# AIRI-Institute/nablaDFT

Measured on AMD Instinct MI355X. Metric: conformer-steps/sec (fwd+bwd) + MAE(E,F) vs CPU reference, higher is better.
Workload: dtype f32 (dense products >= 192 tiles: f32 values split exactly into 3 bf16 pieces, 6 MFMA piece products, f32 accumulate; non-finite operands give NaN where plain f32 gives inf); 1 GPU; PaiNN-OC (nablaDFT/painn_pyg, config/model/painn-oc.yaml: F=128 L=6 R=100 rc=5A K=100) energy+forces train step incl. neighbour list, L1+L2 loss, grad all-reduce, clip 5.0, AdamW lr 5e-4; synthetic ~42-atom drug-like conformers, 2048 conformers/GPU/step; conformers_per_gpu=2048, edges_last_step=1737976, parallelism=dp1

## Files before the change

include/nablaq.h:

```cpp
#ifndef NABLAQ_H
#define NABLAQ_H
#include <stddef.h>
#include <stdint.h>

#ifdef __cplusplus
extern "C" {
#endif

#define NQ_OK 0
#define NQ_ERR_HIP 1
#define NQ_ERR_ARG 2
#define NQ_ERR_MOL_TOO_LARGE 3
#define NQ_ERR_WORKSPACE 4
#define NQ_ERR_NO_EDGES 5

#define NQ_ABI_VERSION 17

typedef struct nq_painn_cfg {
  int32_t hidden_channels;
  int32_t num_layers;
  int32_t num_rbf;
  int32_t num_elements;
  int32_t max_neighbors;
  int32_t envelope_exponent;
// ... 295 lines not shown
void nq_profile_enable(int32_t on);
int nq_profile_read(char* names_host, int32_t name_stride, double* total_ms_host, int64_t* counts_host, int32_t cap);
int nq_profile_read2(char* names_host, int32_t name_stride, double* total_ms_host, int64_t* counts_host, double* flops_host, int32_t cap);

void nq_set_gemm_variant(int32_t variant);
void nq_gemm_splitk_release(void);
int nq_gemm_splitk_state(void* stream, uint64_t* ptr, uint64_t* floats, int32_t* captured, int32_t* retired);

int nq_linear_forward(const float* A, const float* W, const float* bias, float* C, float* C_silu, int32_t M, int32_t N, int32_t K,
                      void* stream);
int nq_linear_forward_act(const float* A, const float* W, float* C, float* C_act, const float* resid, float alpha, float beta, int32_t M, int32_t N,
                          int32_t K, void* stream);
int nq_linear_forward_res(const float* A, const float* W, const float* aux, float alpha, float* C, int32_t M, int32_t N, int32_t K, void* stream);
int nq_bf16_pack(const float* W, int32_t N, int32_t K, void* Wb, void* WbT, void* stream);
int nq_linear_forward_bf16(const float* A, const void* Wb, float* C, float* C_act, const float* resid, float alpha, float beta, int32_t M, int32_t N,
                           int32_t K, void* stream);
int nq_linear_input_grad_bf16(const float* G, const void* WbT, float* C, int32_t M, int32_t N, int32_t K, int32_t accumulate, void* stream);
size_t nq_weight_grad_bf16_scratch_bytes(int64_t rows, int32_t N, int32_t K);
int nq_linear_weight_grad_bf16(const float* G, const float* X, float* gW, int64_t rows, int32_t N, int32_t K, void* scratch, void* stream);
int nq_linear_forward_bf16_out(const void* A, int32_t a_bf16, const void* Wb, void* pre_bf16, void* act, int32_t act_bf16, const float* resid, float alpha,
                               float beta, int32_t M, int32_t N, int32_t K, void* stream);
int nq_linear_weight_grad_bf16_x(const float* G, const void* X_bf16, float* gW, int64_t rows, int32_t N, int32_t K, void* scratch, void* stream);
int nq_gn_ssilu_backward_bf16(const void* z_bf16, const float* g, float scale, int64_t n, float* out, void* stream);
int nq_linear_input_grad(const float* G, const float* W, float* C, int32_t M, int32_t N, int32_t K, int32_t accumulate, void* stream);
int nq_linear_input_grad_epi(const float* G, const float* W, float* C, int32_t M, int32_t N, int32_t K, const float* aux, float alpha, float beta, int32_t mode,
                             void* stream);
int nq_linear_input_grad_bf16_epi(const float* G, const void* WbT, float* C, int32_t M, int32_t N, int32_t K, const float* aux, float alpha, float beta,
                                  int32_t mode, void* stream);
size_t nq_column_sum_scratch_floats(int64_t rows, int32_t cols);
int nq_column_sum(const float* A, int64_t rows, int32_t cols, int64_t lda, float* out, float* scratch, void* stream);
size_t nq_weight_grad_scratch_floats(int64_t rows, int32_t N, int32_t K);
int nq_linear_weight_grad(const float* G, const float* X, float* gW, int64_t rows, int32_t N, int32_t K, float* scratch, void* stream);
int nq_linear_weight_grad_bias(const float* G, const float* X, float* gW, float* gb, int64_t rows, int32_t N, int32_t K, float* scratch, void* stream);

int nq_rccl_available(void);
int nq_rccl_unique_id(void* id128);
int nq_rccl_comm_create(const void* id128, int32_t world, int32_t rank, void** comm);
int nq_rccl_comm_destroy(void* comm);
int nq_rccl_comm_count(void* comm, int32_t* count);
int nq_allreduce(float* buf, size_t n, void* comm, void* stream);
int nq_allreduce_mean(float* buf, size_t n, void* comm, void* stream);
int nq_rccl_broadcast(float* buf, size_t n, int32_t root, void* comm, void* stream);

size_t nq_lbfgs_state_bytes(int32_t N, int32_t B, int32_t memory);
int nq_lbfgs_state_layout(int32_t N, int32_t B, int32_t memory, size_t* offsets_host);
int nq_lbfgs_init(void* state, size_t state_bytes, const int32_t* mol_ptr_host, int32_t N, int32_t B, int32_t memory, const void* pos, int32_t pos_f64,
                  float* pos32, int32_t* n_small_host, void* stream);
int nq_lbfgs_step(void* state, int32_t N, int32_t B, int32_t memory, int32_t n_small, const void* forces, int32_t forces_f64, const uint8_t* fixed_mask,
                  float* pos32, double fmax, double maxstep, double damping, double alpha, int32_t evaluate_only, void* stream);

int nq_md_constants(double* kappa_kb_host);
size_t nq_md_state_bytes(int32_t N, int32_t B, int32_t log_cap, int32_t frame_cap, int32_t flags);
int nq_md_state_layout(int32_t N, int32_t B, int32_t log_cap, int32_t frame_cap, int32_t flags, size_t* offsets_host);
int nq_md_init(void* state, size_t state_bytes, const int32_t* mol_ptr_host, const int64_t* mol_key_host, const double* masses_host, const uint8_t* fixed_host,
               int32_t N, int32_t B, int32_t log_cap, int32_t frame_cap, int32_t flags, const void* pos, int32_t pos_f64, const double* vel, float* pos32,
               int32_t* n_small_host, void* stream);
int nq_md_init_velocities(void* state, int32_t N, int32_t B, int32_t n_small, int32_t log_cap, int32_t frame_cap, int32_t flags, double T_init, int64_t seed,
                          int32_t remove_translation, int32_t remove_rotation, void* stream);
int nq_md_step(void* state, int32_t N, int32_t B, int32_t n_small, int32_t log_cap, int32_t frame_cap, int32_t flags, const void* forces, int32_t forces_f64,
               const void* energies, int32_t energies_f64, float* pos32, int32_t mode, double dt, double kT, double fr, int32_t interval, int64_t seed,
               const double* xi, const double* eta, int32_t finish_only, void* stream);
int nq_md_normals(int64_t seed, int32_t step, int32_t draw, const int32_t* mol_ptr, const int64_t* mol_key, int32_t N, int32_t B, double* out, void* stream);

size_t nq_vib_state_bytes(int32_t N, int32_t B, int32_t D, int64_t P);
int nq_vib_state_layout(int32_t N, int32_t B, int32_t D, int64_t P, size_t* offsets_host);
int nq_vib_init(void* state, size_t state_bytes, const int32_t* mol_ptr_host, const double* masses_host, const uint8_t* fixed_host, int32_t N, int32_t B,
// ... 83 lines not shown
```

nabladft_amd/_lib.py:

```python
import ctypes as C
import os

import torch

_HERE = os.path.dirname(os.path.abspath(__file__))
LIB_PATH = os.environ.get("NABLAQ_LIB") or os.path.join(_HERE, "libnablaq.so")
ABI_VERSION = 17

NQ_OK, NQ_ERR_HIP, NQ_ERR_ARG, NQ_ERR_MOL_TOO_LARGE, NQ_ERR_WORKSPACE, NQ_ERR_NO_EDGES = range(6)


class NablaqError(RuntimeError):
    def __init__(self, code, msg):
        super().__init__(f"libnablaq error {code}: {msg}")
        self.code = code


class PainnCfg(C.Structure):
    _fields_ = [("hidden_channels", C.c_int32), ("num_layers", C.c_int32), ("num_rbf", C.c_int32),
                ("num_elements", C.c_int32), ("max_neighbors", C.c_int32), ("envelope_exponent", C.c_int32),
                ("cutoff", C.c_double), ("rbf_coeff", C.c_float), ("filter_mode", C.c_int32), ("rbf_type", C.c_int32), ("reserved", C.c_int32)]


class SchnetCfg(C.Structure):
# ... 139 lines not shown
    "nq_rowop_blocks": (C.c_int, [_P, _I64, _P, _I64, _P, _I32, _I32, _P, _P, _I64, _I32, _I32, _I32, _I32, _I32, _P]),
    "nq_s2_activation_blocks": (C.c_int, [_P, _P, _I32, _I32, _I32, _I64, _I32, _P, _P, _P, _P, _I32, _P]),
    "nq_column_sum_scratch_floats": (_SZ, [_I64, _I32]),
    "nq_column_sum": (C.c_int, [_P, _I64, _I32, _I64, _P, _P, _P]),
    "nq_es_rotate": (C.c_int, [_P, _I64, _P, _I64, _P, _I32, _P, _P, _I32, _I32, _I64, _P, _I32, _I32, _I32, _P]),
    "nq_es_rotate_back": (C.c_int, [_P, _I64, _I32, _P, _P, _I32, _I32, _P, _P, _P, _P, _I64, _P, _I32, _I32, _I32, _P]),
    "nq_eq_layernorm_forward": (C.c_int, [_P, _I64, _P, _P, _I64, _I32, _F, _P, _I64, _P, _P]),
    "nq_eq_layernorm_scratch_floats": (_SZ, [_I64, _I32]),
    "nq_eq_layernorm_backward": (C.c_int, [_P, _I64, _P, _P, _I64, _P, _I64, _I32, _P, _I64, _P, _P, _P, _P]),
    "nq_eq_norm_sh_forward": (C.c_int, [_P, _P, _P, _P, _P, _I64, _I32, _I32, _F, _P, _P, _P]),
    "nq_eq_norm_sh_scratch_floats": (_SZ, [_I64, _I32, _I32]),
    "nq_eq_norm_sh_backward": (C.c_int, [_P, _P, _P, _P, _P, _P, _I64, _I32, _I32, _P, _P, _P, _P, _P, _P]),
    "nq_eq_logits_forward": (C.c_int, [_P, _P, _I64, _I32, _I32, _P, _P]),
    "nq_eq_logits_scratch_floats": (_SZ, [_I64, _I32, _I32]),
    "nq_eq_logits_backward": (C.c_int, [_P, _P, _P, _I64, _I32, _I32, _P, _P, _P, _P]),
    "nq_eq_softmax_forward": (C.c_int, [_P, _P, _I64, _I32, _P, _P]),
    "nq_eq_softmax_backward": (C.c_int, [_P, _P, _P, _I64, _I32, _P, _P]),
    "nq_eq_head_scale": (C.c_int, [_I32, _P, _P, _P, _P, _I64, _I32, _I32, _P, _P, _P]),
    "nq_eq_scale": (C.c_int, [_P, _P, _P, _P, _I64, _I32, _I32, _P, _P]),
    "nq_loss_l1_l2": (C.c_int, [_P, _P, _I32, _P, _P, _I32, _F, _F, _P, _P, _P, _P]),
    "nq_loss_mse": (C.c_int, [_P, _P, _I32, _P, _P, _I32, _F, _F, _P, _P, _P, _P]),
    "nq_adamw_step": (C.c_int, [_P, _P, _P, _P, _SZ, _F, _F, _F, _F, _F, _F, _I32, _P, _P]),
    "nq_profile_enable": (None, [_I32]),
    "nq_profile_read": (C.c_int, [C.c_char_p, _I32, C.POINTER(C.c_double), C.POINTER(C.c_int64), _I32]),
    "nq_profile_read2": (C.c_int, [C.c_char_p, _I32, C.POINTER(C.c_double), C.POINTER(C.c_int64), C.POINTER(C.c_double), _I32]),
    "nq_set_gemm_variant": (None, [_I32]),
    "nq_gemm_splitk_release": (None, []),
    "nq_gemm_splitk_state": (C.c_int, [_P, C.POINTER(C.c_uint64), C.POINTER(C.c_uint64), C.POINTER(C.c_int32), C.POINTER(C.c_int32)]),
    "nq_linear_forward": (C.c_int, [_P, _P, _P, _P, _P, _I32, _I32, _I32, _P]),
    "nq_linear_input_grad": (C.c_int, [_P, _P, _P, _I32, _I32, _I32, _I32, _P]),
    "nq_weight_grad_scratch_floats": (_SZ, [_I64, _I32, _I32]),
    "nq_linear_weight_grad": (C.c_int, [_P, _P, _P, _I64, _I32, _I32, _P, _P]),
    "nq_linear_weight_grad_bias": (C.c_int, [_P, _P, _P, _P, _I64, _I32, _I32, _P, _P]),
    "nq_rccl_available": (C.c_int, []),
    "nq_rccl_unique_id": (C.c_int, [_P]),
    "nq_rccl_comm_create": (C.c_int, [_P, _I32, _I32, C.POINTER(C.c_void_p)]),
    "nq_rccl_comm_destroy": (C.c_int, [_P]),
    "nq_rccl_comm_count": (C.c_int, [_P, C.POINTER(C.c_int32)]),
    "nq_allreduce": (C.c_int, [_P, _SZ, _P, _P]),
    "nq_allreduce_mean": (C.c_int, [_P, _SZ, _P, _P]),
    "nq_rccl_broadcast": (C.c_int, [_P, _SZ, _I32, _P, _P]),
    "nq_lbfgs_state_bytes": (_SZ, [_I32, _I32, _I32]),
    "nq_lbfgs_state_layout": (C.c_int, [_I32, _I32, _I32, C.POINTER(_SZ)]),
    "nq_lbfgs_init": (C.c_int, [_P, _SZ, _P, _I32, _I32, _I32, _P, _I32, _P, C.POINTER(C.c_int32), _P]),
    "nq_lbfgs_step": (C.c_int, [_P, _I32, _I32, _I32, _I32, _P, _I32, _P, _P, _D, _D, _D, _D, _I32, _P]),
    "nq_md_constants": (C.c_int, [C.POINTER(C.c_double)]),
    "nq_md_state_bytes": (_SZ, [_I32, _I32, _I32, _I32, _I32]),
    "nq_md_state_layout": (C.c_int, [_I32, _I32, _I32, _I32, _I32, C.POINTER(_SZ)]),
    "nq_md_init": (C.c_int, [_P, _SZ, _P, _P, _P, _P, _I32, _I32, _I32, _I32, _I32, _P, _I32, _P, _P, C.POINTER(C.c_int32), _P]),
    "nq_md_init_velocities": (C.c_int, [_P, _I32, _I32, _I32, _I32, _I32, _I32, _D, _I64, _I32, _I32, _P]),
    "nq_md_step": (C.c_int, [_P, _I32, _I32, _I32, _I32, _I32, _I32, _P, _I32, _P, _I32, _P, _I32, _D, _D, _D, _I32, _I64, _P, _P, _I32, _P]),
    "nq_md_normals": (C.c_int, [_I64, _I32, _I32, _P, _P, _I32, _I32, _P, _P]),
    "nq_vib_state_bytes": (_SZ, [_I32, _I32, _I32, _I64]),
    "nq_vib_state_layout": (C.c_int, [_I32, _I32, _I32, _I64, C.POINTER(_SZ)]),
    "nq_vib_init": (C.c_int, [_P, _SZ, _P, _P, _P, _I32, _I32, _I32, _I64, _P, _I32, C.POINTER(C.c_int32), _P]),
    "nq_vib_displace": (C.c_int, [_P, _I32, _I32, _I32, _I64, _I32, _I32, _D, _P, _I64, _P]),
    "nq_vib_accumulate": (C.c_int, [_P, _I32, _I32, _I32, _I64, _I32, _I32, _P, _I32, _I64, _P]),
    "nq_vib_finish": (C.c_int, [_P, _I32, _I32, _I32, _I64, _P]),
    "nq_vib_eigh": (C.c_int, [_P, _I32, _I32, _I32, _I64, _I32, _I32, _I32, _I32, _P]),
    "nq_g3d_max_mol_atoms": (C.c_int32, []),
    "nq_g3d_pair_forward": (C.c_int, [_P] * 9 + [_I32, _I32, _I32, _P, _P, _P, _P, _P]),
    "nq_g3d_pair_scratch_floats": (_SZ, [_I32, _I64, _I32]),
    "nq_g3d_pair_backward": (C.c_int, [_P] * 12 + [_I32, _I64, _I32] + [_P] * 8),
    "nq_g3d_bias_to_heads": (C.c_int, [_P, _P, _P, _P, _I32, _I32, _P, _P]),
    "nq_g3d_bias_from_heads": (C.c_int, [_P, _P, _P, _P, _I32, _I32, _P, _P]),
    "nq_g3d_attention_forward": (C.c_int, [_P, _P, _P, _F, _P, _P, _I32, _I32, _I32, _I32, _I32, _F, _P, _P, _P]),
# ... 106 lines not shown
```

nabladft_amd/build.py:

```python
import os
import subprocess
import sys

HERE = os.path.dirname(os.path.abspath(__file__))
CSRC = os.path.join(HERE, "csrc")
OBJ = os.path.join(HERE, "csrc", "_obj")
LIB = os.path.join(HERE, "libnablaq.so")
SOURCES = ["graph.hip", "gemm.hip", "gemm_bf16.hip", "edge.hip", "molpair.hip", "updfuse.hip", "node.hip", "schnet.hip", "hblock.hip", "so3.hip", "qhnet.hip", "qhgen.hip", "gemnet_graph.hip", "gemnet.hip", "escn.hip", "equiformer.hip", "geobasis.hip", "graphormer.hip", "dimenet.hip", "lbfgs.hip", "md.hip", "vib.hip", "rccl.hip", "engine.hip"]
EXTRA = {"molpair.hip": ["-fno-slp-vectorize"], "md.hip": ["-ffp-contract=off"], "vib.hip": ["-ffp-contract=off"]}
FLAGS = ["--offload-arch=gfx950", "-O3", "-std=c++17", "-fPIC", "-fno-fast-math", "-ffp-contract=on", "-Wall", "-Wno-unused-function"]


def _newer(target, deps):
    if not os.path.exists(target):
        return True
    t = os.path.getmtime(target)
    return any(os.path.getmtime(d) > t for d in deps)


def build(force=False, verbose=True):
    hipcc = os.environ.get("HIPCC", "/opt/rocm/bin/hipcc")
    os.makedirs(OBJ, exist_ok=True)
    headers = [os.path.join(CSRC, "common.h"), os.path.join(CSRC, "lanes.h"), os.path.join(CSRC, "gemm_tile.h"), os.path.join(CSRC, "gemm_split.h"), os.path.join(CSRC, "cg_l4.inc"), os.path.join(os.path.dirname(HERE), "include", "nablaq.h")]
    objs, procs = [], []
    for s in SOURCES:
        src, obj = os.path.join(CSRC, s), os.path.join(OBJ, s.replace(".hip", ".o"))
        objs.append(obj)
        if force or _newer(obj, [src] + headers):
            cmd = [hipcc] + FLAGS + EXTRA.get(s, []) + ["-c", src, "-o", obj]
            if verbose:
                print(" ".join(cmd), flush=True)
            procs.append((s, subprocess.Popen(cmd, stdout=subprocess.PIPE, stderr=subprocess.STDOUT, text=True)))
    failed = False
    for s, p in procs:
        out, _ = p.communicate()
        if out.strip() and verbose:
            print(out)
        if p.returncode != 0:
            print(f"hipcc failed on {s}:\n{out}", file=sys.stderr)
            failed = True
    if failed:
        raise RuntimeError("hipcc compilation failed")
    if force or procs or _newer(LIB, objs):
        cmd = [hipcc, "--offload-arch=gfx950", "-shared", "-fPIC", "-o", LIB] + objs
        if verbose:
            print(" ".join(cmd), flush=True)
        subprocess.check_call(cmd)
    return LIB


if __name__ == "__main__":
    build(force="--force" in sys.argv)
    print("built", LIB)
```

nabladft_amd/csrc/engine.hip:

```cpp
#include <stdarg.h>
#include <stdlib.h>
#include <string.h>

#include "../../include/nablaq.h"
#include "common.h"

thread_local char nq_err_buf[512] = "";
int nq_fail(int code, const char* fmt, ...) {
  va_list ap;
  va_start(ap, fmt);
  vsnprintf(nq_err_buf, sizeof(nq_err_buf), fmt, ap);
  va_end(ap);
  return code;
}

#include <map>
#include <mutex>
#include <utility>
static std::mutex g_lds_mu;
static std::map<std::pair<int, const void*>, size_t> g_lds_granted;
int nq_dyn_lds(const void* kernel, size_t bytes) {
  int dev = 0;
  NQ_HIP(hipGetDevice(&dev));
  std::lock_guard<std::mutex> lock(g_lds_mu);
// ... 93 lines not shown
    y.Z1 = take(2 * N * F); y.Hh = take(2 * N * F); y.XH = take(2 * N * 3 * F);
    y.PHI = take(EP * 3 * F); y.PSI = take(EP * 3 * F); y.WRT = take(R * 3 * F);
    y.XM = take(2 * N * F); y.VM = take(2 * N * 3 * F); y.UU = take(2 * N * 6 * F);
    y.S = take(2 * N * F); y.CAT = take(2 * N * 2 * F); y.ZQ = take(2 * N * F); y.Q = take(2 * N * F); y.Y = take(2 * N * 3 * F);
    y.UFRAG = take(nq_updfuse_frag_floats((int)F));
    const size_t st_ = W->fused ? 1 : 0;
    y.LGY = take(st_ * 2 * N * 3 * F); y.LGCAT = take(st_ * 2 * N * 2 * F); y.LGU = take(st_ * 2 * N * 6 * F); y.LGXH = take(st_ * 2 * N * 3 * F);
    y.LGXA = take(st_ * N * F); y.LGXB = take(st_ * N * F); y.LGVA = take(st_ * N * 3 * F); y.LGVB = take(st_ * N * 3 * F);
    y.LGQ = take(st_ * 2 * N * F); y.LGH = take(st_ * 2 * N * F); y.LGQP = take(st_ * N * F); y.LGHP = take(st_ * N * F);
  }
  W->RHO2 = take(2 * EP * R);
  W->ORDER = take(W->fused ? E : 0);
  W->RW = take(W->fused ? E * 32 : 0);
  W->ZO = take(2 * N * H); W->e_atom = take(N); W->te_atom = take(N);
  W->TD = take(E); W->TR = take(3 * E); W->pos_dot = take(3 * N); W->ge = take(N); W->gte = take(N);
  W->GX = take(2 * N * F); W->GVa = take(2 * N * 3 * F); W->GVb = take(2 * N * 3 * F);
  W->GY = take(2 * N * 3 * F); W->GQ = take(2 * N * F); W->GCAT = take(2 * N * 2 * F); W->GU = take(2 * N * 6 * F);
  W->GXH = take(2 * N * 3 * F); W->GH = take(2 * N * F);
  W->GBR = take(N * 3 * F);
  W->GPHI2 = take(2 * E * 3 * F);
  W->GEDGE = take((F / 64) * E * 4);
  W->GZO = take(2 * N * H); W->TMPW = take(N * H);
  W->GRHO = take(c->rbf_type ? 2 * E * R : 0); W->BCON = take(c->rbf_type ? E * R : 0);
  W->ROWCTR = take(5 * L * NQ_ROWCTR_INTS);
  W->SCHED = take(W->fused ? nq_molgw_sched_ints((int)E, (int)B) : 0);
  W->GWREC = take(W->fused ? nq_molgw_rec_floats((int)E, (int)B) : 0);
  W->GWPART = take(W->fused ? nq_molgw_part_floats((int)F, (int)B) : 0);
  size_t s = 0;
  auto mx = [&](size_t v) { if (v > s) s = v; };
  mx(nq_gemm_tn_scratch_floats(2 * N, 3 * F, F)); mx(nq_gemm_tn_scratch_floats(2 * N, F, 2 * F)); mx(nq_gemm_tn_scratch_floats(6 * N, 2 * F, F));
  mx(W->fused ? nq_gwr_scratch_floats((int)E, (int)F, (int)R) : nq_gemm_tn_scratch_floats(2 * E, 3 * F, R));
  if (W->fused) mx(nq_k0_sort_scratch_ints((int)E, (int)R));
  mx(nq_gemm_tn_scratch_floats(2 * N, F, F)); mx(nq_gemm_tn_scratch_floats(2 * N, H, F));
  mx(nq_colsum_scratch_floats(N > E ? N : E, 3 * F));
  if (c->rbf_type) { mx(nq_colsum_scratch_floats(E, R)); mx(nq_colsum_scratch_floats(E * R, 1)); }
  mx(nq_embed_grad_scratch_floats((int)N, (int)F, (int)T));
  W->scratch_floats = s;
  W->scratch = take(s);
  W->total_floats = o;
  (void)B;
}

enum { GW_PAIR_ROWS = 0, GW_MOLECULE = 1, GW_MIXED = 2 };
struct StepPlan {
  bool fused;
  int gw_mode, gw_cap;
  bool lite;
  bool fused_update;
  bool layer0;
  bool top_layer;
  bool side_fwd, side_geom, side_reduce;
  bool geom_rev_serial;
};
static StepPlan plan_step(const nq_painn_cfg* c, const nq_graph* g, bool want_forces) {
  auto env_on = [](const char* name) { const char* v = getenv(name); return v && v[0] == '1'; };
  StepPlan p{};
  p.fused = c->rbf_type == 0 && nq_filter_fits_lds(c->hidden_channels, c->num_rbf) && !env_on("NQ_NO_FUSED_FILTER");
  const char* cap = getenv("NQ_MOLGW_CAP");
  const int hw = nq_molgw_max_atoms();
  p.gw_cap = cap && atoi(cap) > 0 && atoi(cap) < hw ? atoi(cap) : hw;
  p.gw_mode = GW_PAIR_ROWS;
  if (p.fused && !env_on("NQ_NO_MOLGW") && nq_molgw_config_ok(c->hidden_channels, c->num_rbf) && g->max_mol_atoms > 0 && (env_on("NQ_MOLGW") || g->N >= 4096))
    p.gw_mode = g->max_mol_atoms <= p.gw_cap ? GW_MOLECULE : GW_MIXED;
  p.lite = p.fused && want_forces && !env_on("NQ_NO_LITE");
  p.fused_update = nq_updfuse_frag_floats(c->hidden_channels) > 0 && !env_on("NQ_NO_FUSED_UPDATE") && !nq_gemm_exact_f32_requested();
  p.layer0 = !env_on("NQ_NO_LAYER0");
// ... 520 lines not shown
  NQ_TRY(nq_gemm_nn(st, ws + W.GZO, params + P.O1, ws + W.GX, lite ? N : 2 * N, H, F, H, F, F, 0, "O1"));
  float* gv_cur = ws + W.GVa; float* gv_oth = ws + W.GVb;
  const bool top_layer = plan.top_layer && !seeded;
  if (!top_layer) NQ_HIP(hipMemsetAsync(gv_cur, 0, (lite ? 3 : 6) * NF * sizeof(float), st));
  if (seeded) {
    if (seed_x) NQ_TRY(nq_axpy(st, seed_x, ws + W.GX, (long)NF));
    if (seed_vec) NQ_HIP(hipMemcpyAsync(gv_cur, seed_vec, 3 * NF * sizeof(float), hipMemcpyDeviceToDevice, st));
  }
  float* gphi = ws + W.GPHI2; float* gpsi = gphi + (size_t)E * 3 * F;
  const int* const n_big_pairs = sched + nq_molgw_sched_ints(E, g.B) - 1;
  if (molgw && !geom_aside) NQ_TRY(nq_molgw_geometry(st, g, ws + W.RW, ws + W.TD, ws + W.TR, sched, ws + W.GWREC));
  if (geom_aside) ss.main_waits(geom_ready);
  if (mixed) NQ_HIP(hipMemsetAsync(ws + W.GBR, 0, 3 * NF * sizeof(float), st));
  for (int l = L - 1; l >= 0; --l) {
    const WsLayer& y = W.lay[l]; const MsgP& mp = P.msg[l]; const UpdP& up = P.upd[l];
    const bool top = top_layer && l == L - 1;
    const bool l0 = plan.layer0 && l == 0;
    float* const GYs = lite ? ws + y.LGY : ws + W.GY;
    float* const GCATs = lite ? ws + y.LGCAT : ws + W.GCAT;
    float* const GUs = lite ? ws + y.LGU : ws + W.GU;
    float* const GXHs = lite ? ws + y.LGXH : ws + W.GXH;
    float* const GQs = lite ? ws + y.LGQ : ws + W.GQ;
    float* const GHs = lite ? ws + y.LGH : ws + W.GH;
    UpdRevArgs u{};
    u.N = N; u.F = F; u.U = ws + y.UU; u.Y = ws + y.Y; u.S = ws + y.S; u.CAT = ws + y.CAT;
    u.TU = ws + y.UU + 6 * NF; u.TY = ws + y.Y + 3 * NF; u.TS = ws + y.S + NF; u.TCAT = ws + y.CAT + 2 * NF;
    u.GX = ws + W.GX; u.GTX = lite ? ws + y.LGXA : ws + W.GX + NF; u.GV = gv_cur; u.GTV = lite ? ws + y.LGVA : gv_cur + 3 * NF;
    u.GY = GYs; u.GTY = GYs + 3 * NF; u.GCAT = GCATs; u.GTCAT = GCATs + 2 * NF;
    u.GU = GUs; u.GTU = GUs + 6 * NF;
    u.lite = lite ? 1 : 0;
    ss.before_main_writes(SB_GY);
    NQ_TRY(nq_upd_rev(st, u, 1, true, top));
    sd = ss.fork();
    NQ_TRY(nq_gemm_tn(sd, GYs, ws + y.Q, gp + up.V2, 2L * N, 3 * F, F, 3 * F, F, scr, "V2", gp + up.c2, N));
    ss.read_by_side(SB_GY);
    ss.before_main_writes(SB_GQ);
    NQ_TRY(nq_gemm_nn(st, GYs, params + up.V2, GQs, lite ? N : 2 * N, top ? 2 * F : 3 * F, F, 3 * F, F, F, 0, "V2"));
    NQ_TRY(nq_silu_rev(st, ws + y.ZQ, ws + y.ZQ + NF, GQs, lite ? ws + y.LGQP : GQs + NF, (long)NF, true, lite));
    sd = ss.fork();
    NQ_TRY(nq_gemm_tn(sd, GQs, ws + y.CAT, gp + up.V1, 2L * N, F, 2 * F, F, 2 * F, scr, "V1", gp + up.c1, N));
    ss.read_by_side(SB_GQ);
    NQ_TRY(nq_gemm_nn(st, GQs, params + up.V1, GCATs, lite ? N : 2 * N, F, 2 * F, F, 2 * F, 2 * F, 0, "V1"));
    ss.before_main_writes(SB_GU);
    NQ_TRY(nq_upd_rev(st, u, 2, true, top));
    sd = ss.fork();
    NQ_TRY(nq_gemm_tn(sd, GUs, ws + y.VM, gp + up.U, 6L * N, 2 * F, F, 2 * F, F, scr, "U"));
    ss.read_by_side(SB_GU);
    NQ_TRY(nq_gemm_nn(st, GUs, params + up.U, gv_cur, lite ? 3 * N : 6 * N, 2 * F, F, 2 * F, F, F, top ? 0 : 1, "U"));
    MsgRevArgs m{};
    m.g = g; m.F = F; m.V = ws + W.V[l]; m.XH = ws + y.XH; m.PHI = ws + y.PHI; m.PSI = ws + y.PSI;
    m.TV = ws + W.V[l] + 3 * NF; m.TXH = ws + y.XH + 3 * NF; m.TD = ws + W.TD; m.TR = ws + W.TR;
    m.GX = ws + W.GX; m.GV = gv_cur; m.GTX = lite ? ws + y.LGXB : ws + W.GX + NF; m.GTV = lite ? ws + y.LGVB : gv_cur + 3 * NF;
    m.GXH = GXHs; m.GTXH = GXHs + 3 * NF; m.GV_out = gv_oth; m.GTV_out = gv_oth + 3 * NF;
    m.lite = lite ? 1 : 0;
    m.GPHI = gphi; m.GPSI = gpsi; m.GBR = ws + W.GBR;
    ss.before_main_writes(SB_GXH); ss.before_main_writes(SB_GPHI); ss.before_main_writes(SB_GBR);
    if (W.fused) {
      FilterArgs fa;
      nq_make_filter_args(&fa, ws + y.WRT, params + mp.br, rbf_offsets, ws + W.RW, R, cfg->cutoff, cfg->envelope_exponent, cfg->rbf_coeff, cfg->filter_mode);
      fa.row_ctr = row_ctr(3, l);
      m.mol_cap = plan.gw_cap;
      m.row_filter = mixed ? 1 : 0;
      NQ_TRY(nq_msgf_rev(st, m, fa, true, !molgw, l0));
      if (mixed) {
        m.row_filter = 2;
        fa.row_ctr = row_ctr(4, l);
        NQ_TRY(nq_msgf_rev(st, m, fa, true, true));
// ... 94 lines not shown
```

nabladft_amd/csrc/gemm.hip:

```cpp
#include <algorithm>
#include <map>
#include <mutex>
#include <vector>
#include "gemm_tile.h"
#include "gemm_split.h"

#define BM 128
#define BN 128

__device__ __forceinline__ long rm_row(int q, int w, int ncomp, int base) { return (long)(q / w) * ncomp + base + q % w; }

#define LDS_KC (BM + 1)
#define LDS_MC (BM + 4)

template <bool KC, int NT, int BKT, bool MAP = false>
__device__ __forceinline__ void fetch_tile(float4 (&v)[BM * BKT / 4 / NT], const float* __restrict__ src, int ld, int r0, int R, int k0, int Kend,
                                           bool vec_ok, int mw = 1, int mn = 1, int mb = 0) {
  const int t = threadIdx.x;
#pragma unroll
  for (int it = 0; it < BM * BKT / 4 / NT; ++it) {
    const int idx = t + NT * it;
    float4 x = make_float4(0.f, 0.f, 0.f, 0.f);
    if (KC) {
      const int row = idx / (BKT / 4), kq = (idx % (BKT / 4)) * 4;
      const int gr = r0 + row, gk = k0 + kq;
      if (gr < R) {
        const float* ptr = src + (MAP ? rm_row(gr, mw, mn, mb) : (long)gr) * ld + gk;
        if (vec_ok && gk + 3 < Kend) x = *reinterpret_cast<const float4*>(ptr);
        else {
          if (gk + 0 < Kend) x.x = ptr[0];
          if (gk + 1 < Kend) x.y = ptr[1];
          if (gk + 2 < Kend) x.z = ptr[2];
          if (gk + 3 < Kend) x.w = ptr[3];
        }
      }
    } else {
      const int k = idx >> 5, rq = (idx & 31) * 4;
      const int gk = k0 + k, gr = r0 + rq;
// ... 213 lines not shown
      acc = __builtin_amdgcn_mfma_f32_32x32x2f32(a, b, acc, 0, 0, 0);
    }
    __syncthreads();
  }
  const int col = n0 + wn * 32 + lr;
  if (col >= p.N) return;
  const float bv = p.bias ? p.bias[col] : 0.f;
#pragma unroll
  for (int r = 0; r < 16; ++r) {
    const int row = m0 + wm * 32 + (r & 3) + 8 * (r >> 2) + 4 * lk;
    if (row >= p.M) continue;
    const long off = (long)row * p.ldc + col;
    const float v = acc[r] + bv;
    if (EPI == EPI_ACC) p.C[off] += v;
    else if (EPI == EPI_DSILU) p.C[off] = p.eb * v * nq_dsilu_fast(p.resid[off]);
    else if (EPI == EPI_RES) p.C[off] = p.ea * p.resid[off] + v;
    else p.C[off] = v;
    if (EPI == EPI_SILU) p.C2[off] = nq_silu(v);
    if (EPI == EPI_SILU_RES) p.C2[off] = p.resid ? p.ea * p.resid[off] + p.eb * nq_silu_fast(v) : p.eb * nq_silu_fast(v);
    if (EPI == EPI_DSILU2) p.C2[off] = v * nq_dsilu_fast(p.resid[off]);
  }
}
static bool gemm_is_small(int M, int N) { return (long)nq_cdiv(M, BM) * nq_cdiv(N, BN) < 256; }

enum GemmVariant : int {
  GV_WAVES8 = 1,
  GV_PREFETCH = 2,
  GV_NO_SMALL = 8,
  GV_GENERIC_ONLY = 16,
  GV_EXACT_F32 = 32,
  GV_SPLIT_ALWAYS = 64,
  GV_NO_SPLITK = 128,
  GV_SPH_ROW_MAPPED = 256,
};
static int g_gemm_variant = GV_WAVES8;
extern "C" void nq_set_gemm_variant(int32_t v) { g_gemm_variant = v; }

template <bool A_KC, bool B_KC, int EPI, int BKT = 32>
static void launch_gemm(hipStream_t st, dim3 grid, const GemmArgs& p) {
  int variant = g_gemm_variant & (GV_WAVES8 | GV_PREFETCH);
  if (variant == GV_WAVES8 && (long)grid.x * grid.y * grid.z < 512) variant |= GV_PREFETCH;
  if (variant == GV_WAVES8 && A_KC) variant |= GV_PREFETCH;
  switch (variant) {
    case 0: hipLaunchKernelGGL((k_gemm<A_KC, B_KC, EPI, 4, false, BKT>), grid, dim3(256), 0, st, p); break;
    case GV_WAVES8: hipLaunchKernelGGL((k_gemm<A_KC, B_KC, EPI, 8, false, BKT>), grid, dim3(512), 0, st, p); break;
    case GV_PREFETCH: hipLaunchKernelGGL((k_gemm<A_KC, B_KC, EPI, 4, true, BKT>), grid, dim3(256), 0, st, p); break;
    default: hipLaunchKernelGGL((k_gemm<A_KC, B_KC, EPI, 8, true, BKT>), grid, dim3(512), 0, st, p); break;
  }
}

#define RP_CHUNKS 8
#define RP_ELEMS 32
#define RP_MIN_SPLITS 32
__device__ __forceinline__ float reduce_range(const float* __restrict__ part, long stride, long i, int k, int kend) {
  float s0 = 0.f, s1 = 0.f, s2 = 0.f, s3 = 0.f;
  for (; k + 3 < kend; k += 4) {
    s0 += part[(long)k * stride + i]; s1 += part[(long)(k + 1) * stride + i];
    s2 += part[(long)(k + 2) * stride + i]; s3 += part[(long)(k + 3) * stride + i];
  }
  for (; k < kend; ++k) s0 += part[(long)k * stride + i];
  return (s0 + s1) + (s2 + s3);
}
__device__ __forceinline__ void reduce_partials_body(const float* __restrict__ part, int nsplit, long stride, long count, float* __restrict__ out, long block) {
  if (nsplit < RP_MIN_SPLITS) {
    const long i = block * (RP_CHUNKS * RP_ELEMS) + threadIdx.x;
    if (i < count) out[i] = reduce_range(part, stride, i, 0, nsplit);
// ... 283 lines not shown

int nq_gemm_nn(hipStream_t st, const float* G, const float* W, float* C, int M, int Nout, int Kin, int ldg, int ldw, int ldc,
               int accumulate, const char* tag) {
  GEMM_PROLOGUE(st, "nn", tag, M, Kin, Nout);
  const GemmArgs p = gemm_args(G, W, C, M, Kin, Nout, ldg, ldw, ldc);
  int rc;
  if (try_splitk<true, false>(st, p, nullptr, accumulate, rc)) { NQ_TRY(rc); NQ_LAUNCH_CHECK(); return NQ_OK; }
  return accumulate ? launch_product<true, false, EPI_ACC, 16>(st, p, Nout) : launch_product<true, false, EPI_STORE, 16>(st, p, Nout);
}

int nq_gemm_nn_epi(hipStream_t st, const float* G, const float* W, float* C, int M, int Nout, int Kin, const float* aux, float ea, float eb, int mode, const char* tag, int ldg) {
  GEMM_PROLOGUE(st, "nn", tag, M, Kin, Nout);
  GemmArgs p = gemm_args(G, W, C, M, Kin, Nout, ldg > 0 ? ldg : Nout, Kin, Kin);
  gemm_aux(p, aux, ea, eb);
  return mode == 1 ? launch_product<true, false, EPI_DSILU, 16>(st, p, Nout) : launch_product<true, false, EPI_RES, 16>(st, p, Nout);
}

int nq_gemm_nn_dsilu2(hipStream_t st, const float* G, const float* W, float* C, float* C2, const float* aux, int M, int Nout, int Kin, const char* tag, int ldg) {
  GEMM_PROLOGUE(st, "nn", tag, M, Kin, Nout);
  GemmArgs p = gemm_args(G, W, C, M, Kin, Nout, ldg > 0 ? ldg : Nout, Kin, Kin);
  p.C2 = C2; gemm_aux(p, aux, 0.f, 1.f);
  return launch_product<true, false, EPI_DSILU2, 16>(st, p, Nout);
}

static int tn_splits(long rows, int Mo, int No, int slots) {
  const long tiles = (long)nq_cdiv(Mo, BM) * nq_cdiv(No, BN);
  long s = slots / tiles;
  const long by_rows = (rows + 127) / 128;
  if (s > by_rows) s = by_rows;
  if (s < 1) s = 1;
  return (int)s;
}
static int tn_slots(bool with_bias) { return (gemm3_disabled() || with_bias) ? 512 : 768; }
size_t nq_gemm_tn_scratch_floats(long rows, int Mo, int No) { return (size_t)tn_splits(rows, Mo, No, 768) * ((size_t)Mo * No + Mo); }

int nq_gemm_tn(hipStream_t st, const float* GY, const float* X, float* out, long rows, int Mo, int No, int ldg, int ldx, float* scratch,
               const char* tag, float* bias_out, long bias_rows) {
  GEMM_PROF(st, "gemm_tn:%s[%dx%d]", tag, Mo, No, 2.0 * rows * Mo * No);
  if (rows <= 0) {
    NQ_HIP(hipMemsetAsync(out, 0, sizeof(float) * Mo * No, st));
    if (bias_out) NQ_HIP(hipMemsetAsync(bias_out, 0, sizeof(float) * Mo, st));
    return NQ_OK;
  }
  if (rows > 2000000000L) return nq_fail(NQ_ERR_ARG, "gemm_tn: too many rows");
  int kper = 0, nse = 0;
  float* bpart = nullptr;
  GemmArgs p{};
  auto plan = [&](int slots) {
    const int ns = tn_splits(rows, Mo, No, slots);
    kper = (int)((rows + ns - 1) / ns);
    kper = (kper + 31) / 32 * 32;
    bpart = bias_out ? scratch + (size_t)ns * Mo * No : nullptr;
    p = gemm_args(GY, X, scratch, Mo, No, (int)rows, ldg, ldx, No);
    p.k_per_split = kper; p.part_stride = (long)Mo * No; p.bpart = bpart; p.brows = (int)bias_rows;
    nse = nq_cdiv(rows, kper);
  };
  const int slots0 = tn_slots(bias_out != nullptr);
  plan(slots0);
  if (slots0 != 512 && !gemm3_ok<false, false>(p, kper, nse)) plan(512);
  NQ_TRY((launch_product<false, false, EPI_PARTIAL>(st, p, kper, nse)));
  const long cnt = (long)Mo * No;
  if (bias_out) {
    const unsigned ba = reduce_partials_blocks(nse, cnt), bb = reduce_partials_blocks(nse, (long)Mo);
    hipLaunchKernelGGL(k_reduce_partials2, dim3(ba + bb), dim3(RP_CHUNKS * RP_ELEMS), 0, st, scratch, cnt, out, (int)ba, bpart, (long)Mo, bias_out, nse);
  } else {
    LAUNCH_REDUCE_PARTIALS(st, scratch, nse, cnt, cnt, out);
  }
  NQ_LAUNCH_CHECK();
  return NQ_OK;
}

static int cs_rows_for(long rows) { long c = (rows + 127) / 128; c = (c + 15) / 16 * 16; return (int)(c < 64 ? 64 : (c > CS_ROWS ? CS_ROWS : c)); }
size_t nq_colsum_scratch_floats(long rows, int cols) { const long c = nq_cdiv(rows, cs_rows_for(rows)); return (size_t)(c < 128 ? 128 : c) * cols; }

int nq_colsum(hipStream_t st, const float* A, long rows, int cols, int lda, float* out, float* scratch) {
  NQ_PROF(st, "colsum");
  if (rows <= 0) {
    NQ_HIP(hipMemsetAsync(out, 0, sizeof(float) * cols, st));
    return NQ_OK;
  }
  const int csr = cs_rows_for(rows), chunks = nq_cdiv(rows, csr);
  hipLaunchKernelGGL(k_colsum_partial, dim3(nq_cdiv(cols, 64), chunks), dim3(256), 0, st, A, rows, cols, lda, scratch, csr);
  NQ_LAUNCH_CHECK();
  LAUNCH_REDUCE_PARTIALS(st, scratch, chunks, (long)cols, (long)cols, out);
  NQ_LAUNCH_CHECK();
  return NQ_OK;
}

int nq_reduce_partials(hipStream_t st, const float* part, int nsplit, long stride, long count, float* out) {
  LAUNCH_REDUCE_PARTIALS(st, part, nsplit, stride, count, out);
  NQ_LAUNCH_CHECK();
  return NQ_OK;
}
// ... 54 lines not shown
  return nq_gemm_nt((hipStream_t)stream, A, Wt, C, bias, C_silu, M, N, K, K, K, N);
}
int nq_linear_forward_act(const float* A, const float* Wt, float* C, float* C_act, const float* resid, float alpha, float beta, int32_t M, int32_t N, int32_t K,
                          void* stream) {
  if (!A || !Wt || !C || !C_act) return nq_fail(NQ_ERR_ARG, "null argument");
  return nq_gemm_nt_act((hipStream_t)stream, A, Wt, C, C_act, resid, alpha, beta, M, N, K);
}
int nq_linear_forward_res(const float* A, const float* Wt, const float* aux, float alpha, float* C, int32_t M, int32_t N, int32_t K, void* stream) {
  if (!A || !Wt || !C || !aux) return nq_fail(NQ_ERR_ARG, "null argument");
  if (aux == C) return nq_fail(NQ_ERR_ARG, "nq_linear_forward_res: aux must not alias C");
  return nq_gemm_nt_res((hipStream_t)stream, A, Wt, C, aux, alpha, M, N, K);
}
int nq_linear_input_grad(const float* G, const float* Wt, float* C, int32_t M, int32_t N, int32_t K, int32_t accumulate, void* stream) {
  return nq_gemm_nn((hipStream_t)stream, G, Wt, C, M, N, K, N, K, K, accumulate);
}
int nq_linear_input_grad_epi(const float* G, const float* Wt, float* C, int32_t M, int32_t N, int32_t K, const float* aux, float alpha, float beta, int32_t mode,
                             void* stream) {
  if (!G || !Wt || !C || !aux || (mode != 1 && mode != 2)) return nq_fail(NQ_ERR_ARG, "bad argument");
  return nq_gemm_nn_epi((hipStream_t)stream, G, Wt, C, M, N, K, aux, alpha, beta, mode);
}
size_t nq_column_sum_scratch_floats(int64_t rows, int32_t cols) { return nq_colsum_scratch_floats((long)rows, cols); }
int nq_column_sum(const float* A, int64_t rows, int32_t cols, int64_t lda, float* out, float* scratch, void* stream) {
  if (!A || !out || !scratch || cols < 1 || lda < cols) return nq_fail(NQ_ERR_ARG, "column_sum: bad argument");
  return nq_colsum((hipStream_t)stream, A, (long)rows, cols, (int)lda, out, scratch);
}
size_t nq_weight_grad_scratch_floats(int64_t rows, int32_t N, int32_t K) { return nq_gemm_tn_scratch_floats(rows, N, K); }
int nq_linear_weight_grad(const float* G, const float* X, float* gW, int64_t rows, int32_t N, int32_t K, float* scratch, void* stream) {
  return nq_gemm_tn((hipStream_t)stream, G, X, gW, rows, N, K, N, K, scratch);
}
int nq_linear_weight_grad_bias(const float* G, const float* X, float* gW, float* gb, int64_t rows, int32_t N, int32_t K, float* scratch, void* stream) {
  if (!gb) return nq_fail(NQ_ERR_ARG, "null bias gradient");
  return nq_gemm_tn((hipStream_t)stream, G, X, gW, rows, N, K, N, K, scratch, nullptr, gb, rows);
}

int nq_sph_linear_forward(const float* x, const float* const* W_host, const float* bias0, float* y, int64_t rows, int32_t order, int32_t Fin,
                          int32_t Fout, void* stream) {
  return sph_linear<true>(x, W_host, bias0, y, rows, order, Fin, Fout, "sph_linear_fwd", (hipStream_t)stream);
}

int nq_sph_linear_input_grad(const float* gy, const float* const* W_host, float* gx, int64_t rows, int32_t order, int32_t Fin, int32_t Fout,
                             void* stream) {
  return sph_linear<false>(gy, W_host, nullptr, gx, rows, order, Fin, Fout, "sph_linear_bwd_x", (hipStream_t)stream);
}

size_t nq_sph_weight_grad_scratch_floats(int64_t rows, int32_t order, int32_t Fin, int32_t Fout) {
  const size_t ncomp = (size_t)(order + 1) * (order + 1);
  const size_t sps = sph_tn_splits(rows, (int)ncomp);
  const size_t part = ncomp * sps * (size_t)Fout * Fin + sps * (size_t)Fout, cs = nq_colsum_scratch_floats(rows, Fout);
  return part > cs ? part : cs;
}

int nq_sph_linear_weight_grad(const float* gy, const float* x, float* const* gW_host, float* gbias0, int64_t rows, int32_t order, int32_t Fin,
                              int32_t Fout, float* scratch, void* stream) {
  NQ_TRY(sph_check(rows, order, Fin, Fout));
  if (!gy || !x || !gW_host || !scratch) return nq_fail(NQ_ERR_ARG, "null argument");
  hipStream_t st = (hipStream_t)stream;
  NQ_PROF(st, "sph_linear_bwd_w");
  NQ_PROF_FLOPS(2.0 * rows * (order + 1) * (order + 1) * Fin * Fout);
  const int ncomp = (order + 1) * (order + 1);
  GemmArgs p{};
  for (int L = 0; L <= order; ++L) {
    if (!gW_host[L]) return nq_fail(NQ_ERR_ARG, "null weight gradient");
    if (rows == 0) NQ_HIP(hipMemsetAsync(gW_host[L], 0, sizeof(float) * Fout * Fin, st));
  }
  if (rows > 0) {
    const int sps = sph_tn_splits(rows, ncomp);
// ... 36 lines not shown
```

Measured before the change: 52380 conformer-steps/s.

## Add row-range split-K TN weight-grad kernel and trim top-layer V2 grad

Adds a dedicated TN weight-gradient kernel in which each block owns a contiguous row range and computes the full output tile. It prefetches rows with buffer loads into registers and double-buffers the 3-piece bf16 split in LDS, then writes one partial slab per range, which the existing partials reduction sums. It is used for common PaiNN shapes when the row count is large, and is meant to replace the generic split-K tile launch for these weight-gradient GEMMs. Separately, the top layer's V2 weight grad now computes only the 2F output rows actually used and memsets the rest. The new kernel also raises the scratch requirement.

```diff
diff --git a/include/nablaq.h b/include/nablaq.h
--- a/include/nablaq.h
+++ b/include/nablaq.h
@@ -351,6 +351,8 @@
 size_t nq_weight_grad_scratch_floats(int64_t rows, int32_t N, int32_t K);
 int nq_linear_weight_grad(const float* G, const float* X, float* gW, int64_t rows, int32_t N, int32_t K, float* scratch, void* stream);
 int nq_linear_weight_grad_bias(const float* G, const float* X, float* gW, float* gb, int64_t rows, int32_t N, int32_t K, float* scratch, void* stream);
+int nq_linear_weight_grad_strided(const float* G, const float* X, float* gW, float* gb, int64_t rows, int32_t N, int32_t K, int64_t ldg, int64_t ldx,
+                                  int64_t bias_rows, float* scratch, void* stream);
 
 int nq_rccl_available(void);
 int nq_rccl_unique_id(void* id128);
diff --git a/nabladft_amd/_lib.py b/nabladft_amd/_lib.py
--- a/nabladft_amd/_lib.py
+++ b/nabladft_amd/_lib.py
@@ -195,6 +195,7 @@
     "nq_weight_grad_scratch_floats": (_SZ, [_I64, _I32, _I32]),
     "nq_linear_weight_grad": (C.c_int, [_P, _P, _P, _I64, _I32, _I32, _P, _P]),
     "nq_linear_weight_grad_bias": (C.c_int, [_P, _P, _P, _P, _I64, _I32, _I32, _P, _P]),
+    "nq_linear_weight_grad_strided": (C.c_int, [_P, _P, _P, _P, _I64, _I32, _I32, _I64, _I64, _I64, _P, _P]),
     "nq_rccl_available": (C.c_int, []),
     "nq_rccl_unique_id": (C.c_int, [_P]),
     "nq_rccl_comm_create": (C.c_int, [_P, _I32, _I32, C.POINTER(C.c_void_p)]),
diff --git a/nabladft_amd/build.py b/nabladft_amd/build.py
--- a/nabladft_amd/build.py
+++ b/nabladft_amd/build.py
@@ -21,7 +21,7 @@
 def build(force=False, verbose=True):
     hipcc = os.environ.get("HIPCC", "/opt/rocm/bin/hipcc")
     os.makedirs(OBJ, exist_ok=True)
-    headers = [os.path.join(CSRC, "common.h"), os.path.join(CSRC, "lanes.h"), os.path.join(CSRC, "gemm_tile.h"), os.path.join(CSRC, "gemm_split.h"), os.path.join(CSRC, "cg_l4.inc"), os.path.join(os.path.dirname(HERE), "include", "nablaq.h")]
+    headers = [os.path.join(CSRC, "common.h"), os.path.join(CSRC, "lanes.h"), os.path.join(CSRC, "gemm_tile.h"), os.path.join(CSRC, "gemm_split.h"), os.path.join(CSRC, "gemm_rows.h"), os.path.join(CSRC, "cg_l4.inc"), os.path.join(os.path.dirname(HERE), "include", "nablaq.h")]
     objs, procs = [], []
     for s in SOURCES:
         src, obj = os.path.join(CSRC, s), os.path.join(OBJ, s.replace(".hip", ".o"))
diff --git a/nabladft_amd/csrc/engine.hip b/nabladft_amd/csrc/engine.hip
--- a/nabladft_amd/csrc/engine.hip
+++ b/nabladft_amd/csrc/engine.hip
@@ -149,6 +149,7 @@
   mx(W->fused ? nq_gwr_scratch_floats((int)E, (int)F, (int)R) : nq_gemm_tn_scratch_floats(2 * E, 3 * F, R));
   if (W->fused) mx(nq_k0_sort_scratch_ints((int)E, (int)R));
   mx(nq_gemm_tn_scratch_floats(2 * N, F, F)); mx(nq_gemm_tn_scratch_floats(2 * N, H, F));
+  mx(nq_gemm_tn_scratch_floats(2 * N, 2 * F, F));
   mx(nq_colsum_scratch_floats(N > E ? N : E, 3 * F));
   if (c->rbf_type) { mx(nq_colsum_scratch_floats(E, R)); mx(nq_colsum_scratch_floats(E * R, 1)); }
   mx(nq_embed_grad_scratch_floats((int)N, (int)F, (int)T));
@@ -735,7 +736,13 @@
     ss.before_main_writes(SB_GY);
     NQ_TRY(nq_upd_rev(st, u, 1, true, top));
     sd = ss.fork();
-    NQ_TRY(nq_gemm_tn(sd, GYs, ws + y.Q, gp + up.V2, 2L * N, 3 * F, F, 3 * F, F, scr, "V2", gp + up.c2, N));
+    if (top) {
+      NQ_TRY(nq_gemm_tn(sd, GYs, ws + y.Q, gp + up.V2, 2L * N, 2 * F, F, 3 * F, F, scr, "V2", gp + up.c2, N));
+      NQ_HIP(hipMemsetAsync(gp + up.V2 + (size_t)2 * F * F, 0, (size_t)F * F * sizeof(float), sd));
+      NQ_HIP(hipMemsetAsync(gp + up.c2 + 2 * F, 0, (size_t)F * sizeof(float), sd));
+    } else {
+      NQ_TRY(nq_gemm_tn(sd, GYs, ws + y.Q, gp + up.V2, 2L * N, 3 * F, F, 3 * F, F, scr, "V2", gp + up.c2, N));
+    }
     ss.read_by_side(SB_GY);
     ss.before_main_writes(SB_GQ);
     NQ_TRY(nq_gemm_nn(st, GYs, params + up.V2, GQs, lite ? N : 2 * N, top ? 2 * F : 3 * F, F, 3 * F, F, F, 0, "V2"));
diff --git a/nabladft_amd/csrc/gemm.hip b/nabladft_amd/csrc/gemm.hip
--- a/nabladft_amd/csrc/gemm.hip
+++ b/nabladft_amd/csrc/gemm.hip
@@ -4,6 +4,7 @@
 #include <vector>
 #include "gemm_tile.h"
 #include "gemm_split.h"
+#include "gemm_rows.h"
 
 #define BM 128
 #define BN 128
@@ -283,6 +284,8 @@
   GV_SPLIT_ALWAYS = 64,
   GV_NO_SPLITK = 128,
   GV_SPH_ROW_MAPPED = 256,
+  GV_TN_ROWS_ALWAYS = 512,
+  GV_NO_TN_ROWS = 1024,
 };
 static int g_gemm_variant = GV_WAVES8;
 extern "C" void nq_set_gemm_variant(int32_t v) { g_gemm_variant = v; }
@@ -632,7 +635,43 @@
   return (int)s;
 }
 static int tn_slots(bool with_bias) { return (gemm3_disabled() || with_bias) ? 512 : 768; }
-size_t nq_gemm_tn_scratch_floats(long rows, int Mo, int No) { return (size_t)tn_splits(rows, Mo, No, 768) * ((size_t)Mo * No + Mo); }
+
+#define TN_ROWS_RANGES 256
+#define TN_ROWS_MIN_STEPS 16
+static bool tn_rows_shape(int Mo, int No, bool with_bias) {
+  return (No == 128 && (Mo == 384 || (Mo == 256 && with_bias) || Mo == 128 || Mo == 64)) || (Mo == 128 && No == 256);
+}
+static int tn_rows_ranges(long rows) { const long r = (rows + 15) / 16; return (int)(r < TN_ROWS_RANGES ? r : TN_ROWS_RANGES); }
+static int tn_rows_kper(long rows) { const int nr = tn_rows_ranges(rows); return (int)(((rows + nr - 1) / nr + 15) / 16 * 16); }
+static bool tn_rows_ok(const float* GY, const float* X, long rows, int Mo, int No, int ldg, int ldx, bool with_bias) {
+  if (gemm3_disabled() || (g_gemm_variant & (GV_NO_TN_ROWS | GV_GENERIC_ONLY)) || !tn_rows_shape(Mo, No, with_bias) || rows < 1) return false;
+  if ((reinterpret_cast<uintptr_t>(GY) & 15) || (reinterpret_cast<uintptr_t>(X) & 15) || (ldg & 3) || (ldx & 3) || ldg < Mo || ldx < No) return false;
+  if (((long)tn_rows_kper(rows) + 32) * std::max(ldg, ldx) * 4 >= 0x7fffffffL) return false;
+  return (g_gemm_variant & GV_TN_ROWS_ALWAYS) || rows >= (long)TN_ROWS_RANGES * 16 * TN_ROWS_MIN_STEPS;
+}
+template <int MO, int NO, int WM, bool PLAIN = true>
+static int launch_tn_rows(hipStream_t st, const GemmArgs& p, int nranges) {
+  using T = TnRows<MO, NO, WM>;
+  if (p.bpart || !PLAIN) {
+    NQ_DYN_LDS((k_gemm_tn_rows<MO, NO, WM, true>), T::LDS_BYTES);
+    hipLaunchKernelGGL((k_gemm_tn_rows<MO, NO, WM, true>), dim3((unsigned)nranges), dim3(T::NT), T::LDS_BYTES, st, p);
+  } else if constexpr (PLAIN) {
+    NQ_DYN_LDS((k_gemm_tn_rows<MO, NO, WM, false>), T::LDS_BYTES);
+    hipLaunchKernelGGL((k_gemm_tn_rows<MO, NO, WM, false>), dim3((unsigned)nranges), dim3(T::NT), T::LDS_BYTES, st, p);
+  }
+  return NQ_OK;
+}
+static int launch_tn_rows_shape(hipStream_t st, const GemmArgs& p, int nranges) {
+  if (p.M == 384) return launch_tn_rows<384, 128, 4>(st, p, nranges);
+  if (p.M == 256) return launch_tn_rows<256, 128, 4, false>(st, p, nranges);
+  if (p.N == 256) return launch_tn_rows<128, 256, 2>(st, p, nranges);
+  if (p.M == 128) return launch_tn_rows<128, 128, 4>(st, p, nranges);
+  return launch_tn_rows<64, 128, 2>(st, p, nranges);
+}
+size_t nq_gemm_tn_scratch_floats(long rows, int Mo, int No) {
+  const int rr = tn_rows_shape(Mo, No, true) ? tn_rows_ranges(rows) : 0;
+  return (size_t)std::max(tn_splits(rows, Mo, No, 768), rr) * ((size_t)Mo * No + Mo);
+}
 
 int nq_gemm_tn(hipStream_t st, const float* GY, const float* X, float* out, long rows, int Mo, int No, int ldg, int ldx, float* scratch,
                const char* tag, float* bias_out, long bias_rows) {
@@ -655,10 +694,21 @@
     p.k_per_split = kper; p.part_stride = (long)Mo * No; p.bpart = bpart; p.brows = (int)bias_rows;
     nse = nq_cdiv(rows, kper);
   };
-  const int slots0 = tn_slots(bias_out != nullptr);
-  plan(slots0);
-  if (slots0 != 512 && !gemm3_ok<false, false>(p, kper, nse)) plan(512);
-  NQ_TRY((launch_product<false, false, EPI_PARTIAL>(st, p, kper, nse)));
+  if (tn_rows_ok(GY, X, rows, Mo, No, ldg, ldx, bias_out != nullptr)) {
+    const int nr = tn_rows_ranges(rows);
+    kper = tn_rows_kper(rows);
+    nse = nq_cdiv(rows, kper);
+    bpart = bias_out ? scratch + (size_t)nr * Mo * No : nullptr;
+    p = gemm_args(GY, X, scratch, Mo, No, (int)rows, ldg, ldx, No);
+    p.k_per_split = kper; p.part_stride = (long)Mo * No; p.bpart = bpart; p.brows = (int)bias_rows;
+    NQ_TRY(launch_tn_rows_shape(st, p, nse));
+    NQ_LAUNCH_CHECK();
+  } else {
+    const int slots0 = tn_slots(bias_out != nullptr);
+    plan(slots0);
+    if (slots0 != 512 && !gemm3_ok<false, false>(p, kper, nse)) plan(512);
+    NQ_TRY((launch_product<false, false, EPI_PARTIAL>(st, p, kper, nse)));
+  }
   const long cnt = (long)Mo * No;
   if (bias_out) {
     const unsigned ba = reduce_partials_blocks(nse, cnt), bb = reduce_partials_blocks(nse, (long)Mo);
@@ -779,6 +829,12 @@
   if (!gb) return nq_fail(NQ_ERR_ARG, "null bias gradient");
   return nq_gemm_tn((hipStream_t)stream, G, X, gW, rows, N, K, N, K, scratch, nullptr, gb, rows);
 }
+int nq_linear_weight_grad_strided(const float* G, const float* X, float* gW, float* gb, int64_t rows, int32_t N, int32_t K, int64_t ldg, int64_t ldx,
+                                  int64_t bias_rows, float* scratch, void* stream) {
+  if (!G || !X || !gW || !scratch || N < 1 || K < 1 || ldg < N || ldx < K || ldg > 0x7fffffffL || ldx > 0x7fffffffL || bias_rows < 0)
+    return nq_fail(NQ_ERR_ARG, "weight_grad_strided: bad argument");
+  return nq_gemm_tn((hipStream_t)stream, G, X, gW, rows, N, K, (int)ldg, (int)ldx, scratch, nullptr, gb, bias_rows > rows ? rows : bias_rows);
+}
 
 int nq_sph_linear_forward(const float* x, const float* const* W_host, const float* bias0, float* y, int64_t rows, int32_t order, int32_t Fin,
                           int32_t Fout, void* stream) {
diff --git a/nabladft_amd/csrc/gemm_rows.h b/nabladft_amd/csrc/gemm_rows.h
--- /dev/null
+++ b/nabladft_amd/csrc/gemm_rows.h
@@ -0,0 +1,150 @@
+#pragma once
+#include "gemm_split.h"
+
+template <int MO, int NO, int WM>
+struct TnRows {
+  static constexpr int NWAVE = 8, NT = NWAVE * 64, WN = NWAVE / WM, TM = MO / 32 / WM, TN = NO / 32 / WN;
+  static constexpr int NBLK = (MO + NO) / 64, SLOTS = (2 * NBLK + NWAVE - 1) / NWAVE, FULL_SLOTS = 2 * NBLK / NWAVE;
+  static constexpr int PLANE_A = MO * 32, PLANE_B = NO * 32, BUF = 3 * (PLANE_A + PLANE_B);
+  static constexpr int LDS_BYTES = 2 * BUF + 2 * MO * 4;
+  static constexpr int PD = 2;
+  static_assert(MO % 64 == 0 && NO % 64 == 0 && MO % (32 * WM) == 0 && NO % (32 * WN) == 0 && TM * TN >= 1 && TM * TN <= 6, "bad row-range shape");
+  static_assert(MO <= NT && LDS_BYTES <= 160 * 1024, "bad row-range shape");
+};
+
+template <int MO, int NO, int WM, bool WBIAS>
+__global__ __launch_bounds__(512, 2) void k_gemm_tn_rows(GemmArgs p) {
+  using T = TnRows<MO, NO, WM>;
+  constexpr int SLOTS = T::SLOTS, TM = T::TM, TN = T::TN, PD = T::PD;
+  extern __shared__ __attribute__((aligned(16))) char tn_rows_lds[];
+  char* const lds = tn_rows_lds;
+
+  const int range = blockIdx.x;
+  const int kbeg = range * p.k_per_split, kend = min(p.K, kbeg + p.k_per_split);
+  const int kl = kend - kbeg;
+  if (kl <= 0) return;
+  const int nsteps = (kl + 15) >> 4;
+  const int lane = threadIdx.x & 63, wave = __builtin_amdgcn_readfirstlane((int)(threadIdx.x >> 6));
+  const int kh = wave & 1;
+  const int wm = wave / T::WN, wn = wave % T::WN;
+  const int wrow0 = wm * (TM * 32), wcol0 = wn * (TN * 32);
+  const int lr = lane & 31, lk = lane >> 5;
+
+  __amdgpu_buffer_rsrc_t desc[SLOTS];
+  int ldb4[SLOTS], sto[SLOTS], spl[SLOTS], col0[SLOTS];
+  bool is_a[SLOTS], on[SLOTS];
+#pragma unroll
+  for (int i = 0; i < SLOTS; ++i) {
+    const int blk = (wave >> 1) + 4 * i;
+    on[i] = i < T::FULL_SLOTS || blk < T::NBLK;
+    is_a[i] = blk * 64 < MO;
+    col0[i] = is_a[i] ? blk * 64 : blk * 64 - MO;
+    const int ld = is_a[i] ? p.lda : p.ldb;
+    const float* base = (is_a[i] ? p.A : p.B) + (long)kbeg * ld + col0[i];
+    const long bytes = on[i] ? ((long)(kl - 1) * ld + 64) * 4 : 0L;
+    const unsigned long long b = reinterpret_cast<unsigned long long>(base);
+    const unsigned lo = __builtin_amdgcn_readfirstlane((unsigned)b), hi = __builtin_amdgcn_readfirstlane((unsigned)(b >> 32));
+    const int nrec = __builtin_amdgcn_readfirstlane((int)min(bytes, 0x7fffffffL));
+    desc[i] = __builtin_amdgcn_make_buffer_rsrc(reinterpret_cast<float*>(((unsigned long long)hi << 32) | lo), 0, nrec, 0x00020000);
+    ldb4[i] = __builtin_amdgcn_readfirstlane(ld * 4);
+    sto[i] = (is_a[i] ? 0 : 3 * T::PLANE_A) + (col0[i] + lane) * 32 + kh * 16;
+    spl[i] = is_a[i] ? T::PLANE_A : T::PLANE_B;
+  }
+  const int voff = lane * 4;
+
+  auto fetch = [&](float (&v)[SLOTS][8], int step) {
+    const int krow = __builtin_amdgcn_readfirstlane(min(step, nsteps) * 16 + kh * 8);
+#pragma unroll
+    for (int i = 0; i < SLOTS; ++i)
+#pragma unroll
+      for (int e = 0; e < 8; ++e) v[i][e] = __uint_as_float(__builtin_amdgcn_raw_buffer_load_b32(desc[i], voff, (krow + e) * ldb4[i], 0));
+  };
+  float bsum[SLOTS];
+#pragma unroll
+  for (int i = 0; i < SLOTS; ++i) bsum[i] = 0.f;
+  const bool bias_on = WBIAS && p.bpart != nullptr;
+  auto stash = [&](char* __restrict__ buf, const float (&v)[SLOTS][8], int step) {
+#pragma unroll
+    for (int i = 0; i < SLOTS; ++i) {
+      if (!on[i]) continue;
+      unsigned h[4], m[4], l[4];
+#pragma unroll
+      for (int e = 0; e < 4; ++e) sp_split2<false>(v[i][2 * e], v[i][2 * e + 1], h[e], m[e], l[e]);
+      char* q = buf + sto[i];
+      *reinterpret_cast<gemm_u32x4*>(q) = gemm_u32x4{h[0], h[1], h[2], h[3]};
+      *reinterpret_cast<gemm_u32x4*>(q + spl[i]) = gemm_u32x4{m[0], m[1], m[2], m[3]};
+      *reinterpret_cast<gemm_u32x4*>(q + 2 * spl[i]) = gemm_u32x4{l[0], l[1], l[2], l[3]};
+      if (bias_on && is_a[i]) {
+        const int kb = kbeg + step * 16 + kh * 8;
+        float o = 0.f;
+#pragma unroll
+        for (int e = 0; e < 8; ++e)
+          if (kb + e < p.brows) o += v[i][e];
+        bsum[i] += o;
+      }
+    }
+  };
+
+  f32x16 acc[TM][TN];
+#pragma unroll
+  for (int i = 0; i < TM; ++i)
+#pragma unroll
+    for (int j = 0; j < TN; ++j)
+#pragma unroll
+      for (int r = 0; r < 16; ++r) acc[i][j][r] = 0.f;
+
+  float rg[PD][SLOTS][8];
+#pragma unroll
+  for (int d = 0; d < PD; ++d) fetch(rg[d], d);
+  stash(lds, rg[0], 0);
+  __syncthreads();
+  int s = 0;
+  do {
+#pragma unroll
+    for (int u = 0; u < PD; ++u) {
+      const char* As = lds + (u & 1) * T::BUF;
+      const char* Bs = As + 3 * T::PLANE_A;
+      fetch(rg[u], s + PD);
+      __builtin_amdgcn_sched_barrier(0);
+      {
+        sp_bf8 fa[3][TM], fb[3][TN];
+#pragma unroll
+        for (int pl = 0; pl < 3; ++pl) {
+#pragma unroll
+          for (int i = 0; i < TM; ++i) fa[pl][i] = *reinterpret_cast<const sp_bf8*>(As + pl * T::PLANE_A + (wrow0 + 32 * i + lr) * 32 + lk * 16);
+#pragma unroll
+          for (int j = 0; j < TN; ++j) fb[pl][j] = *reinterpret_cast<const sp_bf8*>(Bs + pl * T::PLANE_B + (wcol0 + 32 * j + lr) * 32 + lk * 16);
+        }
+        constexpr int PA[9] = {2, 2, 1, 1, 2, 0, 1, 0, 0}, PB[9] = {2, 1, 2, 1, 0, 2, 0, 1, 0};
+#pragma unroll
+        for (int tt = 9 - NQ_GEMM3_TERMS; tt < 9; ++tt)
+#pragma unroll
+          for (int i = 0; i < TM; ++i)
+#pragma unroll
+            for (int j = 0; j < TN; ++j) acc[i][j] = __builtin_amdgcn_mfma_f32_32x32x16_bf16(fa[PA[tt]][i], fb[PB[tt]][j], acc[i][j], 0, 0, 0);
+      }
+      stash(lds + ((u + 1) & 1) * T::BUF, rg[(u + 1) % PD], s + 1);
+      ++s;
+      __syncthreads();
+    }
+  } while (s < nsteps);
+
+  float* __restrict__ slab = p.C + (long)range * p.part_stride;
+#pragma unroll
+  for (int i = 0; i < TM; ++i)
+#pragma unroll
+    for (int j = 0; j < TN; ++j)
+#pragma unroll
+      for (int r = 0; r < 16; ++r) slab[(wrow0 + 32 * i + (r & 3) + 8 * (r >> 2) + 4 * lk) * NO + wcol0 + 32 * j + lr] = acc[i][j][r];
+  if (WBIAS) {
+    if (bias_on) {
+      float* lds_b = reinterpret_cast<float*>(lds + 2 * T::BUF);
+#pragma unroll
+      for (int i = 0; i < SLOTS; ++i)
+        if (on[i] && is_a[i]) lds_b[kh * MO + col0[i] + lane] = bsum[i];
+      __syncthreads();
+      const int t = threadIdx.x;
+      if (t < MO) p.bpart[(long)range * MO + t] = lds_b[t] + lds_b[MO + t];
+    }
+  }
+}
```

Result: no change. 52590 conformer-steps/s (median of 6 runs) (+0.4%).
